# Patryk27/strolle

Hardware: NVIDIA H100
Metric: Mrays/s (+ frames/s) at 1080p-per-GPU Cornell, ReSTIR DI+GI + SVGF; H100 vs CPU restatement of the reference (higher is better)
Workload: dtype f32

## Files before the change

### include/strolle_b200.h

```cpp
#ifndef STROLLE_B200_H
#define STROLLE_B200_H

#include <stddef.h>
#include <stdint.h>

#ifdef __cplusplus
extern "C" {
#endif

typedef struct st_engine st_engine;
typedef uint64_t st_handle;
typedef int32_t st_camera_handle;

enum { ST_OK = 0, ST_ERR_CUDA = -1, ST_ERR_INVALID = -2, ST_ERR_NOT_FOUND = -3, ST_ERR_LIMIT = -4 };

typedef struct st_mesh_triangle {
    float positions[3][3];
    float normals[3][3];
    float uvs[3][2];
    float tangents[3][4];
} st_mesh_triangle;

typedef struct st_material {
    float base_color[4];
// ... 63 lines not shown

int st_set_seed_base(st_engine* e, uint32_t base);
int st_set_blue_noise(st_engine* e, const uint8_t* rgba8_256x256);
int st_read_buffer(st_engine* e, st_camera_handle camera, const char* name, float* dst, size_t cap_floats, size_t* count);
int st_read_scene(st_engine* e, const char* name, float* dst, size_t cap_floats, size_t* count);
int st_bvh_depth(st_engine* e, int* depth);
uint32_t st_frame(st_engine* e);
int st_set_frame(st_engine* e, uint32_t frame);
int st_trace_closest(st_engine* e, const float* rays, size_t n, float* out, float* device_ms);
int st_trace_any(st_engine* e, const float* rays, size_t n, uint32_t* out, float* device_ms);
int st_device_math(st_engine* e, int op, const float* a, const float* b, float* out, size_t n);
#define ST_PASS_COUNT 27
int st_enable_timing(st_engine* e, int enabled);
int st_pass_times(st_engine* e, float* ms, uint32_t* launches, int reset);
const char* st_pass_name(int pass);
int st_wavelet_times(st_engine* e, float* ms5, uint32_t* launches5, int reset);
enum { ST_OPT_SVGF_FAST_MATH = 1, ST_OPT_ASYNC_OUTPUT = 2, ST_OPT_HALO_NCCL = 3, ST_OPT_WAVELET_TILED = 4, ST_OPT_WAVELET_TILE_CFG = 5, ST_OPT_FUSE_REPROJECT = 6, ST_OPT_BVH_REUSE = 7, ST_OPT_VARIANCE_TILED = 8, ST_OPT_SHADING_FAST_MATH = 9, ST_OPT_STRIP_FUSED = 10, ST_OPT_FUSED_PASSES = 11, ST_OPT_STRIP_DMA = 12, ST_OPT_WAVELET_PAIRED = 13 };
#define ST_WAVELET_PAIRED_DEFAULT 1
#define ST_STRIP_DMA_DEFAULT (-1)
#define ST_FUSED_PASSES_DEFAULT 1
#define ST_SHADING_FAST_DEFAULT 1
#define ST_VARIANCE_TILED_DEFAULT 1
#define ST_WAVELET_TILED_DEFAULT 15
#define ST_WAVELET_CFG_DEFAULT 0x01000
#define ST_FUSE_REPROJECT_DEFAULT 1
int st_set_option(st_engine* e, int option, int value);
enum { ST_STAT_WAVELET_TILED_LAUNCHES = 1, ST_STAT_WAVELET_TILED_ERRORS = 2, ST_STAT_BVH_GRAFTED_SUBTREES = 3, ST_STAT_VARIANCE_TILED_LAUNCHES = 4,
       ST_STAT_STRIP_PULLED_ROWS = 5 , ST_STAT_LAST_FRAME_FUSED_STRIPS = 6 ,
       ST_STAT_STRIP_FIRST_TIMEOUT = 7  };
int st_get_stat(st_engine* e, int stat, uint64_t* value);
typedef struct st_bvh_builder st_bvh_builder;
int st_bvh_builder_create(st_bvh_builder** out);
void st_bvh_builder_destroy(st_bvh_builder* b);
int st_bvh_builder_build(st_bvh_builder* b, const float* prims11, size_t n, int reuse, float* out, size_t cap_floats, size_t* n_floats,
                         uint32_t* grafted_subtrees, int* depth);
int st_bvh_builder_read(st_bvh_builder* b, float* out, size_t cap_floats);
int st_set_stream(st_engine* e, void* cuda_stream, int external);
int st_count_rays(st_engine* e, int enabled);
int st_ray_count(st_engine* e, uint64_t* rays, int reset);
int st_nccl_unique_id(uint8_t* out128);
int st_nccl_init(st_engine* e, const uint8_t* id128, int rank, int world);
int st_plan_frame(const int* schedule, int n, uint32_t frame, int temporal_reach, char* out, size_t cap);
int st_render_strips(st_engine* e, st_camera_handle camera, void* host_out, int format, int temporal_reach, int gather);
int st_plan_strip_order(const int* schedule, int n, int dma, char* out, size_t cap);
int st_strip_bounds(int height, int world, int* rows_out);
int st_halo_bytes(st_engine* e, uint64_t* bytes);
#define ST_PEER_HANDLE_BYTES 192
int st_peer_export(st_engine* e, st_camera_handle camera, uint8_t* out192);
int st_peer_import(st_engine* e, st_camera_handle camera, const uint8_t* all_handles, int rank, int world);
int st_peer_errors(st_engine* e, st_camera_handle camera, uint32_t* count);
int st_mark_begin(st_engine* e);
int st_mark_end(st_engine* e, float* ms);
// ... 43 lines not shown
```

### rust/strolle-b200-sys/src/lib.rs

```rust
#![allow(non_camel_case_types, clippy::too_many_arguments)]

use std::os::raw::{c_char, c_int, c_void};

#[repr(C)] pub struct st_engine { _private: [u8; 0] }
#[repr(C)] pub struct st_multi { _private: [u8; 0] }
#[repr(C)] pub struct st_bvh_builder { _private: [u8; 0] }
pub type st_handle = u64;
pub type st_camera_handle = i32;

pub const ST_OK: c_int = 0;
pub const ST_ERR_CUDA: c_int = -1;
pub const ST_ERR_INVALID: c_int = -2;
pub const ST_ERR_NOT_FOUND: c_int = -3;
pub const ST_ERR_LIMIT: c_int = -4;

#[repr(C)] #[derive(Clone, Copy, Debug, Default)]
pub struct st_mesh_triangle { pub positions: [[f32; 3]; 3], pub normals: [[f32; 3]; 3], pub uvs: [[f32; 2]; 3], pub tangents: [[f32; 4]; 3] }
#[repr(C)] #[derive(Clone, Copy, Debug, Default)]
pub struct st_material { pub base_color: [f32; 4], pub emissive: [f32; 4], pub perceptual_roughness: f32, pub metallic: f32, pub reflectance: f32, pub ior: f32, pub alpha_blend: i32 }
#[repr(C)] #[derive(Clone, Copy, Debug, Default)]
pub struct st_material_textures { pub base_color: st_handle, pub emissive: st_handle, pub metallic_roughness: st_handle, pub normal_map: st_handle, pub mask: u32 }
pub const ST_LIGHT_POINT: i32 = 1;
pub const ST_LIGHT_SPOT: i32 = 2;
#[repr(C)] #[derive(Clone, Copy, Debug, Default)]
// ... 12 lines not shown
pub const ST_PASS_COUNT: usize = 27;
pub const ST_PEER_HANDLE_BYTES: usize = 192;

pub const ST_OPT_SVGF_FAST_MATH: c_int = 1;
pub const ST_OPT_ASYNC_OUTPUT: c_int = 2;
pub const ST_OPT_HALO_NCCL: c_int = 3;
pub const ST_OPT_WAVELET_TILED: c_int = 4;
pub const ST_OPT_WAVELET_TILE_CFG: c_int = 5;
pub const ST_OPT_FUSE_REPROJECT: c_int = 6;
pub const ST_OPT_BVH_REUSE: c_int = 7;
pub const ST_OPT_VARIANCE_TILED: c_int = 8;
pub const ST_OPT_SHADING_FAST_MATH: c_int = 9;
pub const ST_OPT_STRIP_FUSED: c_int = 10;
pub const ST_OPT_FUSED_PASSES: c_int = 11;
pub const ST_OPT_STRIP_DMA: c_int = 12;
pub const ST_OPT_WAVELET_PAIRED: c_int = 13;
pub const ST_STAT_WAVELET_TILED_LAUNCHES: c_int = 1;
pub const ST_STAT_WAVELET_TILED_ERRORS: c_int = 2;
pub const ST_STAT_BVH_GRAFTED_SUBTREES: c_int = 3;
pub const ST_STAT_VARIANCE_TILED_LAUNCHES: c_int = 4;
pub const ST_STAT_STRIP_PULLED_ROWS: c_int = 5;
pub const ST_STAT_LAST_FRAME_FUSED_STRIPS: c_int = 6;
pub const ST_STAT_STRIP_FIRST_TIMEOUT: c_int = 7;
pub const ST_WAVELET_PAIRED_DEFAULT: c_int = 1;
pub const ST_STRIP_DMA_DEFAULT: c_int = -1;
pub const ST_FUSED_PASSES_DEFAULT: c_int = 1;
pub const ST_SHADING_FAST_DEFAULT: c_int = 1;
pub const ST_VARIANCE_TILED_DEFAULT: c_int = 1;
pub const ST_WAVELET_TILED_DEFAULT: c_int = 15;
pub const ST_WAVELET_CFG_DEFAULT: c_int = 0x01000;
pub const ST_FUSE_REPROJECT_DEFAULT: c_int = 1;

#[link(name = "strolle_b200")]
extern "C" {
    pub fn st_last_error() -> *const c_char;
    pub fn st_engine_create(device: c_int, out: *mut *mut st_engine) -> c_int;
    pub fn st_engine_destroy(e: *mut st_engine);
    pub fn st_insert_mesh(e: *mut st_engine, mesh: st_handle, triangles: *const st_mesh_triangle, count: usize) -> c_int;
    pub fn st_remove_mesh(e: *mut st_engine, mesh: st_handle) -> c_int;
    pub fn st_insert_material(e: *mut st_engine, material: st_handle, m: *const st_material) -> c_int;
    pub fn st_has_material(e: *mut st_engine, material: st_handle) -> c_int;
    pub fn st_remove_material(e: *mut st_engine, material: st_handle) -> c_int;
    pub fn st_insert_image(e: *mut st_engine, image: st_handle, rgba8: *const u8, width: u32, height: u32) -> c_int;
    pub fn st_remove_image(e: *mut st_engine, image: st_handle) -> c_int;
    pub fn st_set_material_textures(e: *mut st_engine, material: st_handle, textures: *const st_material_textures) -> c_int;
    pub fn st_insert_instance(e: *mut st_engine, instance: st_handle, mesh: st_handle, material: st_handle, affine: *const f32) -> c_int;
    pub fn st_remove_instance(e: *mut st_engine, instance: st_handle) -> c_int;
    pub fn st_insert_light(e: *mut st_engine, light: st_handle, l: *const st_light) -> c_int;
    pub fn st_remove_light(e: *mut st_engine, light: st_handle) -> c_int;
    pub fn st_update_sun(e: *mut st_engine, azimuth: f32, altitude: f32) -> c_int;
    pub fn st_create_camera(e: *mut st_engine, camera: *const st_camera, out: *mut st_camera_handle) -> c_int;
    pub fn st_update_camera(e: *mut st_engine, camera: st_camera_handle, desc: *const st_camera) -> c_int;
    pub fn st_delete_camera(e: *mut st_engine, camera: st_camera_handle) -> c_int;
// ... 75 lines not shown
```

### strolle_b200/csrc/engine.cu

```cuda
#include <algorithm>
#include <cmath>
#include <cstdio>
#include <cstring>
#include <deque>
#include <functional>
#include <limits>
#include <string>
#include <unordered_map>
#include <vector>

#include <nccl.h>

#include "../../include/strolle_b200.h"
#include "kernels.h"

#include <dlfcn.h>
namespace {
struct NcclApi {
    void* lib = nullptr;
    ncclResult_t (*GetUniqueId)(ncclUniqueId*) = nullptr;
    ncclResult_t (*CommInitRank)(ncclComm_t*, int, ncclUniqueId, int) = nullptr;
    ncclResult_t (*CommDestroy)(ncclComm_t) = nullptr;
    ncclResult_t (*GroupStart)() = nullptr;
    ncclResult_t (*GroupEnd)() = nullptr;
// ... 356 lines not shown
    std::vector<float4> h_triangles; std::vector<Prim> prims; bool triangles_dirty = false;
    BvhBuild bvh; BvhOut bvh_out; bool bvh_dirty = false;
    std::vector<GpuMaterial> h_materials;
    static const st_handle kSun = ~(st_handle)0;
    std::vector<GpuLight> h_lights; std::vector<std::pair<st_handle, uint32_t>> light_slots;
    std::vector<st_handle> lights_created, lights_updated; std::vector<std::pair<st_handle, uint32_t>> lights_remapped; std::vector<uint32_t> lights_killed;
    uint32_t next_light = 1; bool lights_dirty = true;
    float sun_azimuth = 0.0f, sun_altitude = 0.35f; bool sun_dirty = true;
    GpuWorld world;
    uint32_t frame = 1, seed_base = 0xC0FFEEu;
    DevMem d_triangles, d_bvh, d_materials, d_matpacked, d_unpacklut, d_lights, d_noise, d_tlut, d_slut, d_skylut, d_scratch, d_raycount;
    bool count_rays = false;
    bool svgf_fast = true;
    bool shading_fast = ST_SHADING_FAST_DEFAULT != 0;
    bool fused_passes = ST_FUSED_PASSES_DEFAULT != 0;
    bool async_output = false;
    bool halo_nccl = false;
    int wavelet_paired = ST_WAVELET_PAIRED_DEFAULT;
    int strip_dma = ST_STRIP_DMA_DEFAULT;
    bool strip_fused = true;
    bool last_frame_fused = false;
    int wavelet_tiled = ST_WAVELET_TILED_DEFAULT;
    int wavelet_cfg = ST_WAVELET_CFG_DEFAULT;
    DevMem d_tile_errors; uint64_t wavelet_tiled_launches = 0;
    bool fuse_reproject = ST_FUSE_REPROJECT_DEFAULT != 0;
    bool bvh_reuse = true;
    bool variance_tiled = ST_VARIANCE_TILED_DEFAULT != 0; uint64_t variance_tiled_launches = 0;
    bool luts_static_ready = false, sky_ready = false; float sky_for_altitude = 0.0f;
    std::vector<CameraSlot*> cameras;
    bool timing = false;
    float pass_ms[P_COUNT] = {}; uint32_t pass_launches[P_COUNT] = {};
    float wavelet_ms[5] = {}; uint32_t wavelet_launches[5] = {};
    struct Timed { int pass; cudaEvent_t a, b; int sub; };
    std::vector<Timed> pending; std::vector<cudaEvent_t> event_pool;
    cudaEvent_t mark_a = nullptr, mark_b = nullptr;
    ncclComm_t comm = nullptr; int rank = 0, n_ranks = 1;
    uint64_t halo_bytes_last_frame = 0;

    SceneDev scene() const {
        SceneDev s;
        s.triangles = (const float4*)d_triangles.p; s.bvh = (const float4*)d_bvh.p; s.bvh_len = (uint32_t)bvh_out.buf.size(); s.materials = (const GpuMaterial*)d_materials.p;
        s.lights = (const GpuLight*)d_lights.p; s.blue_noise = (const uchar4*)d_noise.p;
        s.transmittance_lut = (const float4*)d_tlut.p; s.scattering_lut = (const float4*)d_slut.p; s.sky_lut = (const float4*)d_skylut.p;
        s.world = world;
        s.tri_instance = (const uint32_t*)d_tri_instance.p; s.instance_xforms = (const float4*)d_instance_xforms.p;
        s.atlas = (const uchar4*)d_atlas.p; s.srgb_lut = (const float*)d_srgb.p;
        s.material_packed = (const uint32_t*)d_matpacked.p; s.unpack_lut = (const float*)d_unpacklut.p;
// ... 263 lines not shown
    if (d.denoise) {
        if (e->fuse_reproject) {
            add(P_DENOISE_REPROJECT, [=](cudaStream_t s) { launch_denoise_reproject_pair(cam, sc, cur, s); });
        } else {
            add(P_DENOISE_REPROJECT, [=](cudaStream_t s) { launch_denoise_reproject(cam, sc, cur, cam.di_diff_prev_colors, cam.di_diff_moments[cur ^ 1], cam.di_diff_samples, cam.di_diff_curr_colors, cam.di_diff_moments[cur], s); });
            add(P_DENOISE_REPROJECT, [=](cudaStream_t s) { launch_denoise_reproject(cam, sc, cur, cam.gi_diff_prev_colors, cam.gi_diff_moments[cur ^ 1], cam.gi_diff_samples, cam.gi_diff_curr_colors, cam.gi_diff_moments[cur], s); });
        }
        const bool fast = e->svgf_fast;
        const bool var_tiled = e->variance_tiled; uint32_t* verr = (uint32_t*)e->d_tile_errors.p;
        add(P_DENOISE_VARIANCE, [=](cudaStream_t s) {
            if (var_tiled && launch_denoise_variance_tiled(camV, sc, cur, fast, verr, s)) { e->variance_tiled_launches++; return; }
            launch_denoise_variance(camV, sc, cur, fast, s);
        });
        float4* di_io[5][2] = {{cam.di_diff_stash, cam.di_diff_prev_colors}, {cam.di_diff_prev_colors, cam.di_diff_stash}, {cam.di_diff_stash, cam.di_diff_curr_colors},
                               {cam.di_diff_curr_colors, cam.di_diff_stash}, {cam.di_diff_stash, cam.di_diff_curr_colors}};
        float4* gi_io[5][2] = {{cam.gi_diff_stash, cam.gi_diff_prev_colors}, {cam.gi_diff_prev_colors, cam.gi_diff_stash}, {cam.gi_diff_stash, cam.gi_diff_curr_colors},
                               {cam.gi_diff_curr_colors, cam.gi_diff_stash}, {cam.gi_diff_stash, cam.gi_diff_curr_colors}};
        const bool whole_or_fused = ext != nullptr || (cam.y0 == 0 && cam.y1 == cam.h);
        const int first_paired_read = (fast && whole_or_fused && cs->pair[0]) ? (e->wavelet_paired == 2 ? 3 : e->wavelet_paired == 1 ? 4 : 5) : 5;
        for (uint32_t nth = 0; nth < 5; nth++) {
            float4 *a = di_io[nth][0], *b = di_io[nth][1], *c = gi_io[nth][0], *g = gi_io[nth][1];
            const bool reads_pair = (int)nth >= first_paired_read, writes_pair = (int)nth + 1 >= first_paired_read && nth < 4;
            const float4* pin = reads_pair ? cs->pair[nth & 1] : nullptr; float4* pout = writes_pair ? cs->pair[(nth + 1) & 1] : nullptr;
            const bool tiled = !reads_pair && ((e->wavelet_tiled >> nth) & 1) != 0; const int cfg = (e->wavelet_cfg >> (4 * nth)) & 15;
            uint32_t* terr = (uint32_t*)e->d_tile_errors.p;
            const CameraDev camW = grown(cam, x.wavelet[nth]);
            add(P_DENOISE_WAVELET, [=](cudaStream_t s) {
                if (tiled && launch_denoise_wavelet_tiled(camW, sc, f, 1u << nth, (float)(1 + nth), a, b, c, g, pout, fast, cfg, terr, s)) { e->wavelet_tiled_launches++; return; }
                launch_denoise_wavelet(camW, sc, cur, f, 1u << nth, (float)(1 + nth), a, b, c, g, pin, pout, fast, s);
            });
            steps->back().sub = (int)nth;
        }
    }
    uint32_t mode = (uint32_t)d.mode;
    add(P_COMPOSITION, [=](cudaStream_t s) { launch_composition(cam, sc, cur, mode, di_final, gi_final, s); });
}


struct HaloItem { std::string name; int reach; };
struct HaloExchange { int before_step; std::vector<HaloItem> items; };
static const int kSpatialReach = 128;
static const int kPreview2Reach = 64;
static const int kVarianceReach = 3;
static const int kWaveletReach[5] = {1, 2, 4, 9, 19};

static void plan_frame(const int* schedule, int n, uint32_t frame, int temporal_reach, std::vector<HaloExchange>* plan) {
    const char* cur = (frame % 2u == 1u) ? "b" : "a";
    const char* prv = (frame % 2u == 1u) ? "a" : "b";
    bool have_gbuffer = false; int nth_preview = 0, nth_wavelet = 0;
    const char* wavelet_inputs[5] = {"stash", "prev_colors", "stash", "curr_colors", "stash"};
    bool has_preview = false, has_gi_spatial = false;
// ... 759 lines not shown
    std::vector<Prim> all(n);
    uint32_t max_mat = 0;
    for (size_t i = 0; i < n; i++) {
        const float* f = prims11 + 11 * i;
        Prim& p = all[i];
        p.tri = f2bits(f[0]); p.mat = f2bits(f[1]); p.center = h3(f[2], f[3], f[4]);
        p.box.lo = h3(f[5], f[6], f[7]); p.box.hi = h3(f[8], f[9], f[10]);
        max_mat = std::max(max_mat, p.mat);
    }
    b->b.build(all, reuse != 0);
    for (const Prim& p : b->b.prims) max_mat = std::max(max_mat, p.mat);
    std::vector<uint8_t> alpha((size_t)max_mat + 1, 0);
    b->b.flatten(alpha, &b->flat);
    *n_floats = b->flat.buf.size() * 4;
    if (grafted) *grafted = b->b.grafted;
    if (depth) *depth = b->flat.depth;
    if (out) return st_bvh_builder_read(b, out, cap_floats);
    return ST_OK;
}

int st_get_stat(st_engine* e, int stat, uint64_t* value) {
    if (!e || !value) return fail(ST_ERR_INVALID, "null argument");
    if (stat == ST_STAT_WAVELET_TILED_LAUNCHES) { *value = e->wavelet_tiled_launches; return ST_OK; }
    if (stat == ST_STAT_VARIANCE_TILED_LAUNCHES) { *value = e->variance_tiled_launches; return ST_OK; }
    if (stat == ST_STAT_BVH_GRAFTED_SUBTREES) { *value = e->bvh.grafted; return ST_OK; }
    if (stat == ST_STAT_STRIP_PULLED_ROWS) {
        CK(cudaSetDevice(e->device)); CK(cudaStreamSynchronize(e->stream));
        uint64_t total = 0;
        for (CameraSlot* c : e->cameras) if (c->alive && c->peer.sync.p) { uint64_t v = 0; CK(cudaMemcpy(&v, (uint32_t*)c->peer.sync.p + kPulledRowsWord, 8, cudaMemcpyDeviceToHost)); total += v; }
        *value = total; return ST_OK;
    }
    if (stat == ST_STAT_STRIP_FIRST_TIMEOUT) {
        CK(cudaSetDevice(e->device)); CK(cudaStreamSynchronize(e->stream));
        *value = 0;
        for (CameraSlot* c : e->cameras) if (c->alive && c->peer.sync.p && !*value) { uint32_t v = 0; CK(cudaMemcpy(&v, (uint32_t*)c->peer.sync.p + kStripErrorWord + 1, 4, cudaMemcpyDeviceToHost)); *value = v; }
        return ST_OK;
    }
    if (stat == ST_STAT_LAST_FRAME_FUSED_STRIPS) { *value = e->last_frame_fused ? 1 : 0; return ST_OK; }
    if (stat == ST_STAT_WAVELET_TILED_ERRORS) {
        CK(cudaSetDevice(e->device));
        CK(cudaStreamSynchronize(e->stream));
        uint32_t v = 0; CK(cudaMemcpy(&v, e->d_tile_errors.p, 4, cudaMemcpyDeviceToHost));
        *value = v; return ST_OK;
    }
    return fail(ST_ERR_INVALID, "unknown statistic");
}
// ... 414 lines not shown
```

### strolle_b200/csrc/kernels.cu

```cuda
#include <algorithm>
#include <cstdio>
#include <cuda_fp16.h>
#include <cuda.h>
#include <map>
#include <mutex>
#include <tuple>
#include <vector>
#include "st_device.cuh"
#include "kernels.h"

#if defined(ST_FAST) && ST_FAST
#define ST_EXACT_ONLY 0
#else
#define ST_EXACT_ONLY 1
#endif

namespace ST_NS {

#define TILE_W 16
#define TILE_H 8

struct Px { u32 x, y; bool in; };
ST_DEV u32 row_tile(const CameraDev& cam) {
    if (cam.mirror_dn == 0) return blockIdx.y;
// ... 918 lines not shown
                float wd = svgf_luma_weight<false>(scdl, luma(xyz(sdi)), ls_di) * dw * nw;
                if (wd > 0.0f) { sdw += wd; sdc = sdc + wd * xyz(sdi); sdv += sq(wd) * sdi.w; }
                float wg = svgf_luma_weight<false>(scgl, luma(xyz(sgi)), ls_gi) * dw * nw;
                if (wg > 0.0f) { sgw += wg; sgc = sgc + wg * xyz(sgi); sgv += sq(wg) * sgi.w; }
            }
        }
    }
    float4 odi, ogi;
    if (FAST) {
        float rd = sfu_rcp(sdw), rg = sfu_rcp(sgw);
        odi = f4(sdc * rd, sdv * (rd * rd));
        ogi = f4(sgc * rg, sgv * (rg * rg));
    } else {
        odi = f4(sdc / sdw, sdv / (sdw * sdw));
        ogi = f4(sgc / sgw, sgv / (sgw * sgw));
    }
    if (pair_out) st8(pair_out + 2 * i, odi, ogi);
    else { di_out[i] = odi; gi_out[i] = ogi; }
}

ST_DEV u32 smem_addr(const void* p) { return (u32)__cvta_generic_to_shared(p); }
ST_DEV void mbar_init(u32 bar, u32 count) { asm volatile("mbarrier.init.shared::cta.b64 [%0], %1;" ::"r"(bar), "r"(count) : "memory"); }
ST_DEV void mbar_fence_init() { asm volatile("fence.mbarrier_init.release.cluster;" ::: "memory"); }
ST_DEV void mbar_expect_tx(u32 bar, u32 bytes) { asm volatile("mbarrier.arrive.expect_tx.shared::cta.b64 _, [%0], %1;" ::"r"(bar), "r"(bytes) : "memory"); }
ST_DEV bool mbar_try_wait(u32 bar, u32 parity) {
    u32 ok;
    asm volatile("{\n\t.reg .pred p;\n\tmbarrier.try_wait.parity.shared::cta.b64 p, [%1], %2;\n\tselp.u32 %0, 1, 0, p;\n\t}" : "=r"(ok) : "r"(bar), "r"(parity) : "memory");
    return ok != 0u;
}
ST_DEV void tma_load_2d(u32 dst, const CUtensorMap* tm, int c0, int c1, u32 bar) {
    asm volatile("cp.async.bulk.tensor.2d.shared::cluster.global.mbarrier::complete_tx::bytes [%0], [%1, {%2, %3}], [%4];"
                 ::"r"(dst), "l"(reinterpret_cast<unsigned long long>(tm)), "r"(c0), "r"(c1), "r"(bar) : "memory");
}

template <bool FAST> struct WaveletCentre {
    float3 n; float depth, leeway, rcp_leeway, scdl, scgl, ls_di, ls_gi;
    float sdw; float3 sdc; float sdv; float sgw; float3 sgc; float sgv;
    ST_DEV void init(float4 cnd, float4 cdi, float4 cgi, float depth_sigma) {
        n = xyz(cnd); depth = cnd.w; leeway = cnd.w * depth_sigma; rcp_leeway = FAST ? sfu_rcp(leeway) : 0.0f;
        float3 cdc = xyz(cdi), cgc = xyz(cgi);
        scdl = sv_sqrt<FAST>(sv_luma<FAST>(cdc)); scgl = sv_sqrt<FAST>(sv_luma<FAST>(cgc));
        ls_di = lerpc(2.5f, 0.5f, sv_sqrt<FAST>(cdi.w)); ls_gi = lerpc(1.0f, 0.0f, sv_sqrt<FAST>(cgi.w));
        sdw = 1.0f; sdc = cdc; sdv = cdi.w; sgw = 1.0f; sgc = cgc; sgv = cgi.w;
    }
    ST_DEV bool geometry(float4 nds, float* dw, float* nw) const {
        float diff = fabs_(nds.w - depth);
        if (diff >= leeway) return false;
        *dw = FAST ? __fmaf_rn(-diff, rcp_leeway, 1.0f) : 1.0f - diff / leeway;
        *nw = svgf_normal_weight<FAST>(n, xyz(nds));
        return !(*dw == 0.0f || *nw == 0.0f);
    }
    ST_DEV void add(float dw, float nw, float4 sdi, float4 sgi) {
        if (FAST) {
            float dnw = dw * nw;
            float wd = svgf_luma_weight<true>(scdl, sv_luma<true>(xyz(sdi)), ls_di) * dnw;
            if (wd > 0.0f) { sdw += wd; sdc = f3(__fmaf_rn(wd, sdi.x, sdc.x), __fmaf_rn(wd, sdi.y, sdc.y), __fmaf_rn(wd, sdi.z, sdc.z)); sdv = __fmaf_rn(wd * wd, sdi.w, sdv); }
            float wg = svgf_luma_weight<true>(scgl, sv_luma<true>(xyz(sgi)), ls_gi) * dnw;
            if (wg > 0.0f) { sgw += wg; sgc = f3(__fmaf_rn(wg, sgi.x, sgc.x), __fmaf_rn(wg, sgi.y, sgc.y), __fmaf_rn(wg, sgi.z, sgc.z)); sgv = __fmaf_rn(wg * wg, sgi.w, sgv); }
        } else {
            float wd = svgf_luma_weight<false>(scdl, luma(xyz(sdi)), ls_di) * dw * nw;
            if (wd > 0.0f) { sdw += wd; sdc = sdc + wd * xyz(sdi); sdv += sq(wd) * sdi.w; }
            float wg = svgf_luma_weight<false>(scgl, luma(xyz(sgi)), ls_gi) * dw * nw;
            if (wg > 0.0f) { sgw += wg; sgc = sgc + wg * xyz(sgi); sgv += sq(wg) * sgi.w; }
        }
    }
    ST_DEV void store(float4* __restrict__ di_out, float4* __restrict__ gi_out, float4* __restrict__ pair_out, size_t i) const {
        float4 odi, ogi;
        if (FAST) {
            float rd = sfu_rcp(sdw), rg = sfu_rcp(sgw);
            odi = f4(sdc * rd, sdv * (rd * rd));
            ogi = f4(sgc * rg, sgv * (rg * rg));
        } else {
            odi = f4(sdc / sdw, sdv / (sdw * sdw));
            ogi = f4(sgc / sgw, sgv / (sgw * sgw));
        }
        if (pair_out) st8(pair_out + 2 * i, odi, ogi);
        else { di_out[i] = odi; gi_out[i] = ogi; }
    }
};

template <int S, int J, int TW, int TH> struct WaveletTile {
    static constexpr int HL = S + J, BW = TW + 2 * HL, BH = TH + 2 * HL;
    static constexpr u32 BOX_BYTES = (u32)(BW * BH * 16);
    static constexpr u32 PLANE = (BOX_BYTES + 127u) & ~127u;
    static constexpr u32 SMEM = 3u * PLANE + 128u;
};

// ... 41 lines not shown
    const float4* __restrict__ t_gi = reinterpret_cast<const float4*>(s_raw + (base - raw) + 2u * T::PLANE);
    const int c = (ty + T::HL) * T::BW + (tx + T::HL);
    const size_t i = pix(cam, px, py);
    float4 cnd = t_nd[c];
    float4 cdi = t_di[c];
    if (cnd.w == 0.0f) { if (pair_out) pair_out[2 * i] = f4(xyz(cdi), cdi.w); else di_out[i] = f4(xyz(cdi), cdi.w); return; }
    WaveletCentre<FAST> ctr;
    ctr.init(cnd, cdi, t_gi[c], 0.33f / strength);
    const int cj = c + jo;
#pragma unroll
    for (int oy = -1; oy <= 1; oy++) {
#pragma unroll
        for (int ox = -1; ox <= 1; ox++) {
            if (ox == 0 && oy == 0) continue;
            const int k = cj + oy * S * T::BW + ox * S;
            float4 nds = t_nd[k];
            if (nds.w == 0.0f) continue;
            float dw, nw;
            if (!ctr.geometry(nds, &dw, &nw)) continue;
            ctr.add(dw, nw, t_di[k], t_gi[k]);
        }
    }
    ctr.store(di_out, gi_out, pair_out, i);
}

__global__ void __launch_bounds__(ST_BLOCK) k_composition(KPARAMS, int cur, u32 mode, const float4* __restrict__ di_diff, const float4* __restrict__ gi_diff) {
    Px p = pixel_full(cam);
    if (!p.in) return;
    size_t i = pix(cam, p.x, p.y);
    float3 color;
    if (mode == 0u) {
        GBuf g = gbuf_unpack(sc, cam.prim_gbuffer_d0[cur][i], cam.prim_gbuffer_d1[cur][i]);
        float3 dd = xyz(di_diff[i]), ds = xyz(cam.di_spec_samples[i]), gd = xyz(gi_diff[i]), gs = xyz(cam.gi_spec_samples[i]);
        if (g.depth != 0.0f) color = g.emissive + (dd + gd) * xyz(g.base_color) + ds + gs;
        else color = dd;
    } else if (mode == 1u) color = xyz(di_diff[i]);
    else if (mode == 2u) color = xyz(cam.di_spec_samples[i]);
    else if (mode == 3u) color = xyz(gi_diff[i]);
    else if (mode == 4u) color = xyz(cam.gi_spec_samples[i]);
    else if (mode == 5u) color = xyz(cam.ref_colors[i]);
    else if (mode == 6u) { float4 c = cam.ref_colors[i]; color = xyz(c) / c.w; }
    else color = f3s(0.f);
    cam.output[i] = f4(color, 1.0f);
}


// ... 476 lines not shown
    switch (cfg) {
    case 0: return wavelet_tiled_go<FAST, S, J, 32, 8>(c, s, frame, strength, di_in, di_out, gi_in, gi_out, pair_out, errors, st);
    case 1: return wavelet_tiled_go<FAST, S, J, 32, 16>(c, s, frame, strength, di_in, di_out, gi_in, gi_out, pair_out, errors, st);
    case 2: return wavelet_tiled_go<FAST, S, J, 64, 4>(c, s, frame, strength, di_in, di_out, gi_in, gi_out, pair_out, errors, st);
    case 3: return wavelet_tiled_go<FAST, S, J, 64, 8>(c, s, frame, strength, di_in, di_out, gi_in, gi_out, pair_out, errors, st);
    default: return false;
    }
}
bool launch_denoise_wavelet_tiled(const CameraDev& c, const SceneDev& s, u32 frame, u32 stride, float strength, const float4* di_in, float4* di_out, const float4* gi_in,
                                  float4* gi_out, float4* pair_out, bool fast, int cfg, u32* errors, cudaStream_t st) {
    if (c.curr.screen.x != (float)c.w || c.curr.screen.y != (float)c.h) return false;
#define ST_WT(S_, J_) (fast ? wavelet_tiled_cfg<true, S_, J_>(cfg, c, s, frame, strength, di_in, di_out, gi_in, gi_out, pair_out, errors, st) \
                            : wavelet_tiled_cfg<false, S_, J_>(cfg, c, s, frame, strength, di_in, di_out, gi_in, gi_out, pair_out, errors, st))
    switch (stride) {
    case 1: return ST_WT(1, 0);
    case 2: return ST_WT(2, 0);
    case 4: return ST_WT(4, 0);
    case 8: return ST_WT(8, 1);
    case 16: return ST_WT(16, 3);
    default: return false;
    }
#undef ST_WT
}
template <bool FAST>
static bool variance_tiled_go(const CameraDev& c, const SceneDev& s, int cur, u32* errors, cudaStream_t st) {
    typedef VarianceTile<32, 8> T;
    CUtensorMap tn, td, tg;
    if (!wavelet_tensor_map(c.surface_nd, c.w, c.h, T::BW, T::BH, &tn) || !wavelet_tensor_map(c.di_diff_curr_colors, c.w, c.h, T::BW, T::BH, &td) ||
        !wavelet_tensor_map(c.gi_diff_curr_colors, c.w, c.h, T::BW, T::BH, &tg)) return false;
    auto kern = k_denoise_variance_tiled<FAST, 32, 8>;
    static bool attr_set[64] = {};
    int dev = 0; cudaGetDevice(&dev); dev &= 63;
    if (!attr_set[dev]) { if (cudaFuncSetAttribute(kern, cudaFuncAttributeMaxDynamicSharedMemorySize, (int)T::SMEM) != cudaSuccess) { cudaGetLastError(); return false; } attr_set[dev] = true; }
    dim3 grid((c.w + 31) / 32, (c.y1 - c.y0 + 7) / 8);
    kern<<<grid, 256, T::SMEM, st>>>(c, s, cur, tn, td, tg, errors);
    return true;
}
bool launch_denoise_variance_tiled(const CameraDev& c, const SceneDev& s, int cur, bool fast, u32* errors, cudaStream_t st) {
    if (c.curr.screen.x != (float)c.w || c.curr.screen.y != (float)c.h) return false;
    return fast ? variance_tiled_go<true>(c, s, cur, errors, st) : variance_tiled_go<false>(c, s, cur, errors, st);
}
void launch_composition(const CameraDev& c, const SceneDev& s, int cur, u32 mode, const float4* di_diff, const float4* gi_diff, cudaStream_t st) { k_composition<<<grid_full(c), ST_BLOCK, 0, st>>>(c, s, cur, mode, di_diff, gi_diff); }
void launch_output_rgba8(const CameraDev& c, const SceneDev& s, uchar4* out, cudaStream_t st) { k_output_rgba8<<<grid_full(c), ST_BLOCK, 0, st>>>(c, s, out); }
void launch_ref_tracing(const CameraDev& c, const SceneDev& s, u32 depth, cudaStream_t st) { k_ref_tracing<<<grid_full(c), ST_BLOCK, 0, st>>>(c, s, depth); }
void launch_ref_shading(const CameraDev& c, const SceneDev& s, u32 seed, u32 depth, cudaStream_t st) { k_ref_shading<<<grid_full(c), ST_BLOCK, 0, st>>>(c, s, seed, depth); }
void launch_bvh_heatmap(const CameraDev& c, const SceneDev& s, cudaStream_t st) { k_bvh_heatmap<<<grid_full(c), ST_BLOCK, 0, st>>>(c, s); }
// ... 135 lines not shown
```

### strolle_b200/csrc/kernels.h

```cpp
#pragma once
#include <cuda_runtime.h>
#include "st_types.h"

namespace st {
typedef uint32_t u32;

void launch_prim_gbuffer(const CameraDev& c, const SceneDev& s, int cur, int with_reprojection, cudaStream_t st);
void launch_frame_reprojection(const CameraDev& c, const SceneDev& s, int cur, cudaStream_t st);
void launch_di_sampling(const CameraDev& c, const SceneDev& s, int cur, u32 seed, u32 frame, cudaStream_t st);
void launch_di_temporal(const CameraDev& c, const SceneDev& s, int cur, u32 seed, cudaStream_t st);
void launch_di_spatial_pick(const CameraDev& c, const SceneDev& s, int cur, u32 seed, u32 frame, cudaStream_t st);
void launch_spatial_trace(const CameraDev& c, const SceneDev& s, const float4* d0, const float4* d1, float4* d2, cudaStream_t st);
void launch_di_spatial_sample(const CameraDev& c, const SceneDev& s, u32 seed, u32 frame, cudaStream_t st);
void launch_di_resolving(const CameraDev& c, const SceneDev& s, int cur, cudaStream_t st);
void launch_gi_reprojection(const CameraDev& c, const SceneDev& s, int cur, cudaStream_t st);
void launch_gi_sampling_a(const CameraDev& c, const SceneDev& s, int cur, u32 seed, u32 frame, cudaStream_t st);
void launch_gi_sampling_b(const CameraDev& c, const SceneDev& s, int cur, u32 seed, u32 frame, cudaStream_t st);
void launch_gi_temporal(const CameraDev& c, const SceneDev& s, int cur, u32 seed, u32 frame, int inline_reprojection, cudaStream_t st);
void launch_gi_spatial_pick(const CameraDev& c, const SceneDev& s, int cur, u32 seed, u32 frame, cudaStream_t st);
void launch_gi_spatial_sample(const CameraDev& c, const SceneDev& s, u32 seed, u32 frame, cudaStream_t st);
void launch_gi_preview(const CameraDev& c, const SceneDev& s, int cur, u32 seed, u32 nth, const float4* in, float4* out, int mirror_reach, cudaStream_t st);
void launch_gi_resolving(const CameraDev& c, const SceneDev& s, int cur, const float4* in, cudaStream_t st);
void launch_di_sample_temporal(const CameraDev& c, const SceneDev& s, int cur, u32 seed_sampling, u32 seed_temporal, u32 frame, cudaStream_t st);
void launch_di_spatial_fused(const CameraDev& c, const SceneDev& s, int cur, u32 seed_pick, u32 seed_sample, u32 frame, cudaStream_t st);
void launch_gi_sampling_fused(const CameraDev& c, const SceneDev& s, int cur, u32 seed_a, u32 seed_b, u32 frame, cudaStream_t st);
void launch_gi_spatial_fused(const CameraDev& c, const SceneDev& s, int cur, u32 seed_pick, u32 seed_sample, u32 frame, cudaStream_t st);
void launch_gi_preview_resolve(const CameraDev& c, const SceneDev& s, int cur, u32 seed, const float4* in, const float4* source, cudaStream_t st);
void launch_denoise_reproject(const CameraDev& c, const SceneDev& s, int cur, const float4* pc, const float4* pm, const float4* smp, float4* col, float4* mom, cudaStream_t st);
void launch_denoise_reproject_pair(const CameraDev& c, const SceneDev& s, int cur, cudaStream_t st);
void launch_denoise_variance(const CameraDev& c, const SceneDev& s, int cur, bool fast, cudaStream_t st);
void launch_denoise_wavelet(const CameraDev& c, const SceneDev& s, int cur, u32 frame, u32 stride, float strength, const float4* di_in, float4* di_out, const float4* gi_in, float4* gi_out, const float4* pair_in, float4* pair_out, bool fast, cudaStream_t st);
bool launch_denoise_wavelet_tiled(const CameraDev& c, const SceneDev& s, u32 frame, u32 stride, float strength, const float4* di_in, float4* di_out, const float4* gi_in, float4* gi_out, float4* pair_out, bool fast, int cfg, u32* errors, cudaStream_t st);
bool launch_denoise_variance_tiled(const CameraDev& c, const SceneDev& s, int cur, bool fast, u32* errors, cudaStream_t st);
void launch_composition(const CameraDev& c, const SceneDev& s, int cur, u32 mode, const float4* di_diff, const float4* gi_diff, cudaStream_t st);
void launch_output_rgba8(const CameraDev& c, const SceneDev& s, uchar4* out, cudaStream_t st);
void launch_ref_tracing(const CameraDev& c, const SceneDev& s, u32 depth, cudaStream_t st);
void launch_ref_shading(const CameraDev& c, const SceneDev& s, u32 seed, u32 depth, cudaStream_t st);
void launch_bvh_heatmap(const CameraDev& c, const SceneDev& s, cudaStream_t st);
void launch_trace_stream_closest(const SceneDev& s, const float4* rays, long n, float4* out, cudaStream_t st);
void launch_trace_stream_any(const SceneDev& s, const float4* rays, long n, u32* out, cudaStream_t st);
void launch_math(int op, const float* a, const float* b, float* out, long n, cudaStream_t st);
void launch_material_derive(const GpuMaterial* mats, u32 n, u32* packed, cudaStream_t st);
void launch_srgb_lut(float* lut, cudaStream_t st);
void launch_unpack_lut(float* lut, cudaStream_t st);
void launch_atm_transmittance(float4* out, cudaStream_t st);
void launch_atm_scattering(const float4* tl, float4* out, cudaStream_t st);
void launch_atm_sky(const float4* tl, const float4* sl, float sun_altitude, float4* out, cudaStream_t st);

#define ST_PEER_MAX_SEGMENTS 40
#define ST_PEER_MAX_RANKS 16
struct PeerSegment { const uint4* src; uint4* dst; unsigned long long n; };
struct PeerExchange {
    PeerSegment seg[ST_PEER_MAX_SEGMENTS]; int nseg;
    u32* peer_flags[ST_PEER_MAX_RANKS];
    const u32* my_flags;
// ... 53 lines not shown
```

### strolle_b200/engine.py

```python
import ctypes as C
import os

import numpy as np

_HERE = os.path.dirname(os.path.abspath(__file__))
PASS_COUNT = 27
FORMAT_RGBA32F, FORMAT_RGBA8_SRGB = 0, 1
OPT_SVGF_FAST_MATH = 1
OPT_ASYNC_OUTPUT = 2
OPT_HALO_NCCL = 3
OPT_WAVELET_TILED = 4
OPT_WAVELET_TILE_CFG = 5
OPT_FUSE_REPROJECT = 6
OPT_BVH_REUSE = 7
OPT_VARIANCE_TILED = 8
OPT_FUSED_PASSES = 11
OPT_WAVELET_PAIRED = 13
OPT_STRIP_DMA = 12
OPT_STRIP_FUSED = 10
OPT_SHADING_FAST_MATH = 9
WAVELET_TILED_DEFAULT = 15
STAT_WAVELET_TILED_LAUNCHES = 1
STAT_WAVELET_TILED_ERRORS = 2
STAT_BVH_GRAFTED_SUBTREES = 3
STAT_VARIANCE_TILED_LAUNCHES = 4
STAT_STRIP_PULLED_ROWS = 5
STAT_LAST_FRAME_FUSED_STRIPS = 6
STAT_STRIP_FIRST_TIMEOUT = 7


class StrolleError(RuntimeError):
    pass


def lib_path():
    return os.environ.get("STROLLE_B200_LIB") or os.path.join(_HERE, "_lib", "libstrolle_b200.so")


class _MeshTriangle(C.Structure):
    _fields_ = [("positions", C.c_float * 9), ("normals", C.c_float * 9), ("uvs", C.c_float * 6), ("tangents", C.c_float * 12)]


class _Material(C.Structure):
    _fields_ = [("base_color", C.c_float * 4), ("emissive", C.c_float * 4), ("perceptual_roughness", C.c_float), ("metallic", C.c_float),
                ("reflectance", C.c_float), ("ior", C.c_float), ("alpha_blend", C.c_int32)]


class _MaterialTextures(C.Structure):
    _fields_ = [("base_color", C.c_uint64), ("emissive", C.c_uint64), ("metallic_roughness", C.c_uint64), ("normal_map", C.c_uint64), ("mask", C.c_uint32)]


# ... 544 lines not shown
```

Baseline: 3642.

## Add TMA-pipelined vertical sweep kernel for wide-stride SVGF wavelet passes

Adds a wavelet kernel in which each block walks a column band down a segment of rows. A producer warp streams row batches through a shared-memory ring using TMA and mbarriers while the consumer threads filter, so halo rows are reused across steps instead of being reloaded per tile. The default wavelet config now selects this path for the stride-8 pass (nth=3 requires the tiled bit, which default 15 sets), while stride 16 keeps its previous path. It adds producer/consumer sync complexity, timeout error paths, and segment sizing tied to the SM count.

```diff
diff --git a/include/strolle_b200.h b/include/strolle_b200.h
--- a/include/strolle_b200.h
+++ b/include/strolle_b200.h
@@ -109,12 +109,13 @@
 #define ST_SHADING_FAST_DEFAULT 1
 #define ST_VARIANCE_TILED_DEFAULT 1
 #define ST_WAVELET_TILED_DEFAULT 15
-#define ST_WAVELET_CFG_DEFAULT 0x01000
+#define ST_WAVELET_CFG_DEFAULT 0x05000
 #define ST_FUSE_REPROJECT_DEFAULT 1
 int st_set_option(st_engine* e, int option, int value);
 enum { ST_STAT_WAVELET_TILED_LAUNCHES = 1, ST_STAT_WAVELET_TILED_ERRORS = 2, ST_STAT_BVH_GRAFTED_SUBTREES = 3, ST_STAT_VARIANCE_TILED_LAUNCHES = 4,
        ST_STAT_STRIP_PULLED_ROWS = 5 , ST_STAT_LAST_FRAME_FUSED_STRIPS = 6 ,
-       ST_STAT_STRIP_FIRST_TIMEOUT = 7  };
+       ST_STAT_STRIP_FIRST_TIMEOUT = 7 ,
+       ST_STAT_WAVELET_SWEEP_LAUNCHES = 8  };
 int st_get_stat(st_engine* e, int stat, uint64_t* value);
 typedef struct st_bvh_builder st_bvh_builder;
 int st_bvh_builder_create(st_bvh_builder** out);
diff --git a/rust/strolle-b200-sys/src/lib.rs b/rust/strolle-b200-sys/src/lib.rs
--- a/rust/strolle-b200-sys/src/lib.rs
+++ b/rust/strolle-b200-sys/src/lib.rs
@@ -58,13 +58,14 @@
 pub const ST_STAT_STRIP_PULLED_ROWS: c_int = 5;
 pub const ST_STAT_LAST_FRAME_FUSED_STRIPS: c_int = 6;
 pub const ST_STAT_STRIP_FIRST_TIMEOUT: c_int = 7;
+pub const ST_STAT_WAVELET_SWEEP_LAUNCHES: c_int = 8;
 pub const ST_WAVELET_PAIRED_DEFAULT: c_int = 1;
 pub const ST_STRIP_DMA_DEFAULT: c_int = -1;
 pub const ST_FUSED_PASSES_DEFAULT: c_int = 1;
 pub const ST_SHADING_FAST_DEFAULT: c_int = 1;
 pub const ST_VARIANCE_TILED_DEFAULT: c_int = 1;
 pub const ST_WAVELET_TILED_DEFAULT: c_int = 15;
-pub const ST_WAVELET_CFG_DEFAULT: c_int = 0x01000;
+pub const ST_WAVELET_CFG_DEFAULT: c_int = 0x05000;
 pub const ST_FUSE_REPROJECT_DEFAULT: c_int = 1;
 
 #[link(name = "strolle_b200")]
diff --git a/strolle_b200/csrc/engine.cu b/strolle_b200/csrc/engine.cu
--- a/strolle_b200/csrc/engine.cu
+++ b/strolle_b200/csrc/engine.cu
@@ -402,7 +402,7 @@
     bool last_frame_fused = false;
     int wavelet_tiled = ST_WAVELET_TILED_DEFAULT;
     int wavelet_cfg = ST_WAVELET_CFG_DEFAULT;
-    DevMem d_tile_errors; uint64_t wavelet_tiled_launches = 0;
+    DevMem d_tile_errors; uint64_t wavelet_tiled_launches = 0, wavelet_sweep_launches = 0;
     bool fuse_reproject = ST_FUSE_REPROJECT_DEFAULT != 0;
     bool bvh_reuse = true;
     bool variance_tiled = ST_VARIANCE_TILED_DEFAULT != 0; uint64_t variance_tiled_launches = 0;
@@ -712,11 +712,17 @@
             float4 *a = di_io[nth][0], *b = di_io[nth][1], *c = gi_io[nth][0], *g = gi_io[nth][1];
             const bool reads_pair = (int)nth >= first_paired_read, writes_pair = (int)nth + 1 >= first_paired_read && nth < 4;
             const float4* pin = reads_pair ? cs->pair[nth & 1] : nullptr; float4* pout = writes_pair ? cs->pair[(nth + 1) & 1] : nullptr;
-            const bool tiled = !reads_pair && ((e->wavelet_tiled >> nth) & 1) != 0; const int cfg = (e->wavelet_cfg >> (4 * nth)) & 15;
+            const bool tiled_bit = ((e->wavelet_tiled >> nth) & 1) != 0; const int cfg = (e->wavelet_cfg >> (4 * nth)) & 15;
+            const bool tiled = !reads_pair && tiled_bit, sweep = tiled_bit && (cfg == 4 || cfg == 5), long_only = cfg == 5;
+            const int tile_cfg = cfg == 5 ? 1 : cfg;
             uint32_t* terr = (uint32_t*)e->d_tile_errors.p;
             const CameraDev camW = grown(cam, x.wavelet[nth]);
             add(P_DENOISE_WAVELET, [=](cudaStream_t s) {
-                if (tiled && launch_denoise_wavelet_tiled(camW, sc, f, 1u << nth, (float)(1 + nth), a, b, c, g, pout, fast, cfg, terr, s)) { e->wavelet_tiled_launches++; return; }
+                if (sweep && launch_denoise_wavelet_sweep(camW, sc, f, 1u << nth, (float)(1 + nth), a, b, c, g, pin, pout, fast, long_only, terr, s)) {
+                    if (pin) e->wavelet_sweep_launches++; else e->wavelet_tiled_launches++;
+                    return;
+                }
+                if (tiled && launch_denoise_wavelet_tiled(camW, sc, f, 1u << nth, (float)(1 + nth), a, b, c, g, pout, fast, tile_cfg, terr, s)) { e->wavelet_tiled_launches++; return; }
                 launch_denoise_wavelet(camW, sc, cur, f, 1u << nth, (float)(1 + nth), a, b, c, g, pin, pout, fast, s);
             });
             steps->back().sub = (int)nth;
@@ -1522,6 +1528,7 @@
 int st_get_stat(st_engine* e, int stat, uint64_t* value) {
     if (!e || !value) return fail(ST_ERR_INVALID, "null argument");
     if (stat == ST_STAT_WAVELET_TILED_LAUNCHES) { *value = e->wavelet_tiled_launches; return ST_OK; }
+    if (stat == ST_STAT_WAVELET_SWEEP_LAUNCHES) { *value = e->wavelet_sweep_launches; return ST_OK; }
     if (stat == ST_STAT_VARIANCE_TILED_LAUNCHES) { *value = e->variance_tiled_launches; return ST_OK; }
     if (stat == ST_STAT_BVH_GRAFTED_SUBTREES) { *value = e->bvh.grafted; return ST_OK; }
     if (stat == ST_STAT_STRIP_PULLED_ROWS) {
diff --git a/strolle_b200/csrc/kernels.cu b/strolle_b200/csrc/kernels.cu
--- a/strolle_b200/csrc/kernels.cu
+++ b/strolle_b200/csrc/kernels.cu
@@ -964,6 +964,7 @@
 ST_DEV u32 smem_addr(const void* p) { return (u32)__cvta_generic_to_shared(p); }
 ST_DEV void mbar_init(u32 bar, u32 count) { asm volatile("mbarrier.init.shared::cta.b64 [%0], %1;" ::"r"(bar), "r"(count) : "memory"); }
 ST_DEV void mbar_fence_init() { asm volatile("fence.mbarrier_init.release.cluster;" ::: "memory"); }
+ST_DEV void mbar_arrive(u32 bar) { asm volatile("mbarrier.arrive.shared::cta.b64 _, [%0];" ::"r"(bar) : "memory"); }
 ST_DEV void mbar_expect_tx(u32 bar, u32 bytes) { asm volatile("mbarrier.arrive.expect_tx.shared::cta.b64 _, [%0], %1;" ::"r"(bar), "r"(bytes) : "memory"); }
 ST_DEV bool mbar_try_wait(u32 bar, u32 parity) {
     u32 ok;
@@ -992,19 +993,29 @@
         *nw = svgf_normal_weight<FAST>(n, xyz(nds));
         return !(*dw == 0.0f || *nw == 0.0f);
     }
-    ST_DEV void add(float dw, float nw, float4 sdi, float4 sgi) {
+    ST_DEV void weights(float dw, float nw, float4 sdi, float4 sgi, float* wd, float* wg) const {
         if (FAST) {
             float dnw = dw * nw;
-            float wd = svgf_luma_weight<true>(scdl, sv_luma<true>(xyz(sdi)), ls_di) * dnw;
+            *wd = svgf_luma_weight<true>(scdl, sv_luma<true>(xyz(sdi)), ls_di) * dnw;
+            *wg = svgf_luma_weight<true>(scgl, sv_luma<true>(xyz(sgi)), ls_gi) * dnw;
+        } else {
+            *wd = svgf_luma_weight<false>(scdl, luma(xyz(sdi)), ls_di) * dw * nw;
+            *wg = svgf_luma_weight<false>(scgl, luma(xyz(sgi)), ls_gi) * dw * nw;
+        }
+    }
+    ST_DEV void accumulate(float wd, float wg, float4 sdi, float4 sgi) {
+        if (FAST) {
             if (wd > 0.0f) { sdw += wd; sdc = f3(__fmaf_rn(wd, sdi.x, sdc.x), __fmaf_rn(wd, sdi.y, sdc.y), __fmaf_rn(wd, sdi.z, sdc.z)); sdv = __fmaf_rn(wd * wd, sdi.w, sdv); }
-            float wg = svgf_luma_weight<true>(scgl, sv_luma<true>(xyz(sgi)), ls_gi) * dnw;
             if (wg > 0.0f) { sgw += wg; sgc = f3(__fmaf_rn(wg, sgi.x, sgc.x), __fmaf_rn(wg, sgi.y, sgc.y), __fmaf_rn(wg, sgi.z, sgc.z)); sgv = __fmaf_rn(wg * wg, sgi.w, sgv); }
         } else {
-            float wd = svgf_luma_weight<false>(scdl, luma(xyz(sdi)), ls_di) * dw * nw;
             if (wd > 0.0f) { sdw += wd; sdc = sdc + wd * xyz(sdi); sdv += sq(wd) * sdi.w; }
-            float wg = svgf_luma_weight<false>(scgl, luma(xyz(sgi)), ls_gi) * dw * nw;
             if (wg > 0.0f) { sgw += wg; sgc = sgc + wg * xyz(sgi); sgv += sq(wg) * sgi.w; }
         }
+    }
+    ST_DEV void add(float dw, float nw, float4 sdi, float4 sgi) {
+        float wd, wg;
+        weights(dw, nw, sdi, sgi, &wd, &wg);
+        accumulate(wd, wg, sdi, sgi);
     }
     ST_DEV void store(float4* __restrict__ di_out, float4* __restrict__ gi_out, float4* __restrict__ pair_out, size_t i) const {
         float4 odi, ogi;
@@ -1092,6 +1103,129 @@
         }
     }
     ctr.store(di_out, gi_out, pair_out, i);
+}
+
+template <int S, int J, int WB, int RB, int NB> struct WaveletSweep {
+    static constexpr int HL = S + J, BW = WB + 2 * HL, BWH = BW / 2, R = NB * RB, CONSUMERS = WB * RB, THREADS = CONSUMERS + 32;
+    static constexpr int NEED = (RB + 2 * HL - 1) / RB + 1;
+    static constexpr u32 ROW = (u32)BW * 16u;
+    static constexpr u32 PLANE = (u32)R * ROW;
+    static constexpr u32 BATCH_BYTES = 3u * (u32)RB * ROW;
+    static constexpr u32 SMEM = 3u * PLANE + 128u;
+    static_assert(NB >= NEED + 1, "the ring must hold one batch beyond what a step reads");
+    static_assert(BW % 2 == 0 && 2 * BW <= 256 && RB <= 256, "tensor-copy box: at most 256 elements per dimension");
+    static_assert(SMEM + 16u * NB <= 232448u, "shared memory per block on sm_90a");
+};
+
+template <bool FAST, bool PAIR_IN, int S, int J, int WB, int RB, int NB>
+__global__ void __launch_bounds__(WB * RB + 32, 1) k_denoise_wavelet_sweep(KPARAMS, u32 frame, float strength, int seg_rows,
+                                                                     const __grid_constant__ CUtensorMap tm_nd, const __grid_constant__ CUtensorMap tm_a,
+                                                                     const __grid_constant__ CUtensorMap tm_b,
+                                                                     float4* __restrict__ di_out, float4* __restrict__ gi_out, float4* __restrict__ pair_out,
+                                                                     u32* __restrict__ errors) {
+    typedef WaveletSweep<S, J, WB, RB, NB> T;
+    extern __shared__ unsigned char s_raw[];
+    __shared__ __align__(8) unsigned long long s_full[NB], s_empty[NB];
+    const int x0 = (int)blockIdx.x * WB, y0 = cam.y0 + (int)blockIdx.y * seg_rows, y1 = min(y0 + seg_rows, cam.y1);
+    if (y0 >= y1) return;
+    const int steps = (y1 - y0 + RB - 1) / RB, batches = (y1 - y0 - 1 + 2 * T::HL) / RB + 1;
+    const u32 raw = smem_addr(s_raw);
+    const u32 base = (raw + 127u) & ~127u;
+    const unsigned char* sm = s_raw + (base - raw);
+    if (threadIdx.x == 0) {
+        for (int b = 0; b < NB; b++) { mbar_init(smem_addr(&s_full[b]), 1u); mbar_init(smem_addr(&s_empty[b]), (u32)T::CONSUMERS); }
+        mbar_fence_init();
+    }
+    __syncthreads();
+    if ((int)threadIdx.x >= T::CONSUMERS) {
+        if (threadIdx.x != (unsigned)T::CONSUMERS) return;
+        for (int b = 0; b < batches; b++) {
+            const u32 full = smem_addr(&s_full[b % NB]), off = (u32)(b % NB) * (u32)RB * T::ROW;
+            if (b >= NB) {
+                bool done = false;
+                const u32 empty = smem_addr(&s_empty[b % NB]), parity = (u32)(b / NB - 1) & 1u;
+                for (u32 spin = 0; spin < (1u << 20) && !done; spin++) done = mbar_try_wait(empty, parity);
+                if (!done) { atomicAdd(errors, 1u); return; }
+            }
+            const int y = y0 - T::HL + b * RB;
+            mbar_expect_tx(full, T::BATCH_BYTES);
+            tma_load_2d(base + off, &tm_nd, (x0 - T::HL) * 2, y, full);
+            if (PAIR_IN) {
+                tma_load_2d(base + T::PLANE + off, &tm_a, (x0 - T::HL) * 4, y, full);
+                tma_load_2d(base + 2u * T::PLANE + off, &tm_a, (x0 - T::HL + T::BWH) * 4, y, full);
+            } else {
+                tma_load_2d(base + T::PLANE + off, &tm_a, (x0 - T::HL) * 2, y, full);
+                tma_load_2d(base + 2u * T::PLANE + off, &tm_b, (x0 - T::HL) * 2, y, full);
+            }
+        }
+        return;
+    }
+    const float4* __restrict__ r_nd = reinterpret_cast<const float4*>(sm);
+    auto signals = [&](int row, int col, float4* di, float4* gi) {
+        if (PAIR_IN) {
+            const int h = col >= T::BWH ? 1 : 0;
+            const float4* p = reinterpret_cast<const float4*>(sm + (1 + h) * T::PLANE) + 2 * (row * T::BWH + col - h * T::BWH);
+            *di = p[0]; *gi = p[1];
+        } else {
+            *di = reinterpret_cast<const float4*>(sm + T::PLANE)[row * T::BW + col];
+            *gi = reinterpret_cast<const float4*>(sm + 2u * T::PLANE)[row * T::BW + col];
+        }
+    };
+    const int tx = (int)threadIdx.x % WB, ty = (int)threadIdx.x / WB;
+    const u32 px = (u32)(x0 + tx);
+    const float depth_sigma = 0.33f / strength;
+    int landed = 0;
+    bool failed = false;
+    for (int k = 0; k < steps; k++) {
+        const u32 py = (u32)(y0 + k * RB + ty);
+        const bool in = px < (u32)cam.w && py < (u32)y1;
+        int jx = 0, jy = 0;
+        if (in) {
+            float4 bn = blue_noise(sc, px, py, frame);
+            float2 jf = (f2(bn.z, bn.w) - f2(0.5f, 0.5f)) * ((float)S - 1.0f) * 0.5f;
+            jx = to_i32_sat(jf.x); jy = to_i32_sat(jf.y);
+        }
+        for (const int upto = min(k + T::NEED, batches); landed < upto && !failed; landed++) {
+            bool done = false;
+            const u32 bar = smem_addr(&s_full[landed % NB]), parity = (u32)(landed / NB) & 1u;
+            for (u32 spin = 0; spin < (1u << 20) && !done; spin++) done = mbar_try_wait(bar, parity);
+            failed = !done;
+        }
+        if (__any_sync(0xffffffffu, failed)) { if ((threadIdx.x & 31u) == 0u) atomicAdd(errors, 1u); return; }
+        if (in) {
+            const int qc = (k * RB + ty + T::HL) % T::R;
+            const int c = qc * T::BW + tx + T::HL;
+            const size_t i = pix(cam, px, py);
+            float4 cnd = r_nd[c];
+            float4 cdi, cgi;
+            signals(qc, tx + T::HL, &cdi, &cgi);
+            if (cnd.w == 0.0f) { if (pair_out) pair_out[2 * i] = f4(xyz(cdi), cdi.w); else di_out[i] = f4(xyz(cdi), cdi.w); }
+            else {
+                WaveletCentre<FAST> ctr;
+                ctr.init(cnd, cdi, cgi, depth_sigma);
+                float4 tdi[8], tgi[8]; float twd[8], twg[8];
+#pragma unroll
+                for (int t = 0; t < 8; t++) {
+                    const int oy = (t < 3) ? -1 : (t < 5 ? 0 : 1), ox = (t < 3) ? t - 1 : (t < 5 ? (t == 3 ? -1 : 1) : t - 6);
+                    int r = qc + jy + oy * S;
+                    r = r < 0 ? r + T::R : (r >= T::R ? r - T::R : r);
+                    const int col = tx + T::HL + jx + ox * S;
+                    const float4 nds = r_nd[r * T::BW + col];
+                    signals(r, col, &tdi[t], &tgi[t]);
+                    const float diff = fabs_(nds.w - ctr.depth);
+                    const float dw = FAST ? __fmaf_rn(-diff, ctr.rcp_leeway, 1.0f) : 1.0f - diff / ctr.leeway;
+                    const float d = FAST ? __fmaf_rn(nds.z, ctr.n.z, __fmaf_rn(nds.y, ctr.n.y, nds.x * ctr.n.x)) : dot(xyz(nds), ctr.n);
+                    const float x1 = rmax(d, 0.0f), x2 = x1 * x1, x4 = x2 * x2, x8 = x4 * x4, x16 = x8 * x8, x32 = x16 * x16, nw = x32 * x32;
+                    const bool ok = nds.w != 0.0f && !(diff >= ctr.leeway) && !(dw == 0.0f || nw == 0.0f);
+                    ctr.weights(ok ? dw : 0.0f, ok ? nw : 0.0f, tdi[t], tgi[t], &twd[t], &twg[t]);
+                }
+#pragma unroll
+                for (int t = 0; t < 8; t++) ctr.accumulate(twd[t], twg[t], tdi[t], tgi[t]);
+                ctr.store(di_out, gi_out, pair_out, i);
+            }
+        }
+        mbar_arrive(smem_addr(&s_empty[k % NB]));
+    }
 }
 
 __global__ void __launch_bounds__(ST_BLOCK) k_composition(KPARAMS, int cur, u32 mode, const float4* __restrict__ di_diff, const float4* __restrict__ gi_diff) {
@@ -1614,6 +1748,38 @@
     }
 #undef ST_WT
 }
+template <bool FAST, bool PAIR_IN, int S, int J, int WB, int RB, int NB>
+static bool wavelet_sweep_go(const CameraDev& c, const SceneDev& s, u32 frame, float strength, const float4* di_in, float4* di_out, const float4* gi_in, float4* gi_out,
+                             const float4* pair_in, float4* pair_out, bool long_only, u32* errors, cudaStream_t st) {
+    typedef WaveletSweep<S, J, WB, RB, NB> T;
+    static int sms[64] = {};
+    int dev = 0; cudaGetDevice(&dev); dev &= 63;
+    if (!sms[dev] && cudaDeviceGetAttribute(&sms[dev], cudaDevAttrMultiProcessorCount, dev) != cudaSuccess) { cudaGetLastError(); return false; }
+    const int bands = (c.w + WB - 1) / WB, rows = c.y1 - c.y0, steps = (rows + RB - 1) / RB;
+    const int segs = std::max(1, std::min(steps, sms[dev] / bands));
+    const int seg_rows = (steps + segs - 1) / segs * RB;
+    if (long_only && seg_rows < 8 * T::HL) return false;
+    CUtensorMap tn, ta, tb;
+    if (!wavelet_tensor_map(c.surface_nd, c.w, c.h, T::BW, RB, &tn)) return false;
+    if (PAIR_IN) { if (!wavelet_tensor_map(pair_in, 2 * c.w, c.h, T::BW, RB, &ta)) return false; tb = ta; }
+    else if (!wavelet_tensor_map(di_in, c.w, c.h, T::BW, RB, &ta) || !wavelet_tensor_map(gi_in, c.w, c.h, T::BW, RB, &tb)) return false;
+    auto kern = k_denoise_wavelet_sweep<FAST, PAIR_IN, S, J, WB, RB, NB>;
+    static bool attr_set[64] = {};
+    if (!attr_set[dev]) { if (cudaFuncSetAttribute(kern, cudaFuncAttributeMaxDynamicSharedMemorySize, (int)T::SMEM) != cudaSuccess) { cudaGetLastError(); return false; } attr_set[dev] = true; }
+    dim3 grid(bands, (rows + seg_rows - 1) / seg_rows);
+    kern<<<grid, T::THREADS, T::SMEM, st>>>(c, s, frame, strength, seg_rows, tn, ta, tb, di_out, gi_out, pair_out, errors);
+    return true;
+}
+bool launch_denoise_wavelet_sweep(const CameraDev& c, const SceneDev& s, u32 frame, u32 stride, float strength, const float4* di_in, float4* di_out, const float4* gi_in,
+                                  float4* gi_out, const float4* pair_in, float4* pair_out, bool fast, bool long_only, u32* errors, cudaStream_t st) {
+    if (c.curr.screen.x != (float)c.w || c.curr.screen.y != (float)c.h) return false;
+#define ST_WS(F_, P_) (stride == 8 ? wavelet_sweep_go<F_, P_, 8, 1, 88, 4, 8>(c, s, frame, strength, di_in, di_out, gi_in, gi_out, pair_in, pair_out, long_only, errors, st) \
+                                   : wavelet_sweep_go<F_, P_, 16, 3, 44, 8, 7>(c, s, frame, strength, di_in, di_out, gi_in, gi_out, pair_in, pair_out, long_only, errors, st))
+    if (stride != 8 && stride != 16) return false;
+    if (pair_in) return fast ? ST_WS(true, true) : ST_WS(false, true);
+    return fast ? ST_WS(true, false) : ST_WS(false, false);
+#undef ST_WS
+}
 template <bool FAST>
 static bool variance_tiled_go(const CameraDev& c, const SceneDev& s, int cur, u32* errors, cudaStream_t st) {
     typedef VarianceTile<32, 8> T;
diff --git a/strolle_b200/csrc/kernels.h b/strolle_b200/csrc/kernels.h
--- a/strolle_b200/csrc/kernels.h
+++ b/strolle_b200/csrc/kernels.h
@@ -31,6 +31,7 @@
 void launch_denoise_variance(const CameraDev& c, const SceneDev& s, int cur, bool fast, cudaStream_t st);
 void launch_denoise_wavelet(const CameraDev& c, const SceneDev& s, int cur, u32 frame, u32 stride, float strength, const float4* di_in, float4* di_out, const float4* gi_in, float4* gi_out, const float4* pair_in, float4* pair_out, bool fast, cudaStream_t st);
 bool launch_denoise_wavelet_tiled(const CameraDev& c, const SceneDev& s, u32 frame, u32 stride, float strength, const float4* di_in, float4* di_out, const float4* gi_in, float4* gi_out, float4* pair_out, bool fast, int cfg, u32* errors, cudaStream_t st);
+bool launch_denoise_wavelet_sweep(const CameraDev& c, const SceneDev& s, u32 frame, u32 stride, float strength, const float4* di_in, float4* di_out, const float4* gi_in, float4* gi_out, const float4* pair_in, float4* pair_out, bool fast, bool long_only, u32* errors, cudaStream_t st);
 bool launch_denoise_variance_tiled(const CameraDev& c, const SceneDev& s, int cur, bool fast, u32* errors, cudaStream_t st);
 void launch_composition(const CameraDev& c, const SceneDev& s, int cur, u32 mode, const float4* di_diff, const float4* gi_diff, cudaStream_t st);
 void launch_output_rgba8(const CameraDev& c, const SceneDev& s, uchar4* out, cudaStream_t st);
diff --git a/strolle_b200/engine.py b/strolle_b200/engine.py
--- a/strolle_b200/engine.py
+++ b/strolle_b200/engine.py
@@ -27,6 +27,7 @@
 STAT_STRIP_PULLED_ROWS = 5
 STAT_LAST_FRAME_FUSED_STRIPS = 6
 STAT_STRIP_FIRST_TIMEOUT = 7
+STAT_WAVELET_SWEEP_LAUNCHES = 8
 
 
 class StrolleError(RuntimeError):
```

Measured after the change: 3671 (median of 6 runs). No clear change (+0.8%).
